# maturk/dn-splatter

Measured on NVIDIA H100. Metric: rendered Mpix/s (fwd+bwd, RGB+depth+normal), higher is better.
Workload: dtype f32

## Files before the change

dn_splatter_b200/csrc/adam.cu:

```cuda
#include "common.cuh"

namespace {

struct AdamSegDev {
  float* p; const float* g; float* m; float* v;
  int64_t n;
  float step_size, bc2_sqrt, eps;
};

struct AdamLaunch {
  AdamSegDev seg[DNR_ADAM_MAX_SEGS];
  float beta2, w1, w2;
};

__device__ __forceinline__ void adam_one(float& p, float g, float& m, float& v, float w1, float b2, float w2, float step_size,
                                         float bc2_sqrt, float eps) {
  m = m + w1 * (g - m);
  v = b2 * v + w2 * g * g;
  const float denom = sqrtf(v) / bc2_sqrt + eps;
  p = p - step_size * (m / denom);
}

__global__ void __launch_bounds__(256) adam_kernel(const AdamLaunch L) {
  const AdamSegDev& s = L.seg[blockIdx.y];
  const float w1 = L.w1, b2 = L.beta2, w2 = L.w2;
  const float step_size = s.step_size, bc2_sqrt = s.bc2_sqrt, eps = s.eps;
  const int64_t n = s.n;
  const int64_t tid = (int64_t)blockIdx.x * blockDim.x + threadIdx.x, stride = (int64_t)gridDim.x * blockDim.x;
  const bool vec = ((((uintptr_t)s.p | (uintptr_t)s.g | (uintptr_t)s.m | (uintptr_t)s.v) & 15) == 0);
  const int64_t n4 = vec ? (n >> 2) : 0;
  float4* p4 = reinterpret_cast<float4*>(s.p);
  const float4* g4 = reinterpret_cast<const float4*>(s.g);
  float4* m4 = reinterpret_cast<float4*>(s.m);
  float4* v4 = reinterpret_cast<float4*>(s.v);
  for (int64_t i = tid; i < n4; i += stride) {
    float4 p = p4[i], m = m4[i], v = v4[i];
    const float4 g = g4[i];
    adam_one(p.x, g.x, m.x, v.x, w1, b2, w2, step_size, bc2_sqrt, eps);
    adam_one(p.y, g.y, m.y, v.y, w1, b2, w2, step_size, bc2_sqrt, eps);
    adam_one(p.z, g.z, m.z, v.z, w1, b2, w2, step_size, bc2_sqrt, eps);
    adam_one(p.w, g.w, m.w, v.w, w1, b2, w2, step_size, bc2_sqrt, eps);
    p4[i] = p; m4[i] = m; v4[i] = v;
  }
  for (int64_t i = (n4 << 2) + tid; i < n; i += stride) {
    float p = s.p[i], m = s.m[i], v = s.v[i];
    adam_one(p, s.g[i], m, v, w1, b2, w2, step_size, bc2_sqrt, eps);
    s.p[i] = p; s.m[i] = m; s.v[i] = v;
  }
}

struct PeerDev {
  const float* flat[DNR_PEER_MAX];
  const uint8_t* touched[DNR_PEER_MAX];
  int world;
};

__global__ void __launch_bounds__(256) peer_mask_kernel(const PeerDev P, int n, uint8_t* __restrict__ mask) {
  const int i = (blockIdx.x * blockDim.x + threadIdx.x) * 16;
  if (i >= n) return;
  if (i + 16 <= n) {
    uint32_t m[4] = {0u, 0u, 0u, 0u};
    for (int k = 0; k < P.world; ++k) {
      const uint4 t = *reinterpret_cast<const uint4*>(P.touched[k] + i);
      const uint32_t w[4] = {t.x, t.y, t.z, t.w};
#pragma unroll
      for (int j = 0; j < 4; ++j) {
        const uint32_t nz = ((w[j] | ((w[j] & 0x7f7f7f7fu) + 0x7f7f7f7fu)) >> 7) & 0x01010101u;
        m[j] |= nz << k;
      }
    }
    *reinterpret_cast<uint4*>(mask + i) = make_uint4(m[0], m[1], m[2], m[3]);
  } else {
    for (int j = i; j < n; ++j) {
      uint32_t m = 0;
      for (int k = 0; k < P.world; ++k) m |= (P.touched[k][j] ? 1u : 0u) << k;
      mask[j] = (uint8_t)m;
    }
  }
}

struct AdamReduceLaunch {
  AdamLaunch adam;
  int dense[DNR_ADAM_MAX_SEGS];
  int64_t off[DNR_ADAM_MAX_SEGS];
  int32_t width[DNR_ADAM_MAX_SEGS];
};

template <int WORLD>
__global__ void __launch_bounds__(256, WORLD > 4 ? 3 : (WORLD > 1 ? 4 : 5)) adam_reduce_kernel(const AdamReduceLaunch L, const PeerDev P, const uint8_t* __restrict__ mask) {
  const AdamSegDev& s = L.adam.seg[blockIdx.y];
  const float w1 = L.adam.w1, b2 = L.adam.beta2, w2 = L.adam.w2;
  const float step_size = s.step_size, bc2_sqrt = s.bc2_sqrt, eps = s.eps;
  const int64_t n = s.n, off = L.off[blockIdx.y];
  const uint32_t width = (uint32_t)L.width[blockIdx.y];
  const uint32_t all_ranks = L.dense[blockIdx.y] ? ((1u << P.world) - 1u) : 0u;
  const int64_t tid = (int64_t)blockIdx.x * blockDim.x + threadIdx.x, stride = (int64_t)gridDim.x * blockDim.x;
  const int64_t n4 = n >> 2;
  float4* p4 = reinterpret_cast<float4*>(s.p);
  float4* m4 = reinterpret_cast<float4*>(s.m);
  float4* v4 = reinterpret_cast<float4*>(s.v);
  for (int64_t i = tid; i < n4; i += stride) {
    const uint32_t e = (uint32_t)(i << 2);
    uint32_t mk = all_ranks | (uint32_t)mask[e / width] | (uint32_t)mask[(e + 1u) / width] |
                  (uint32_t)mask[(e + 2u) / width] | (uint32_t)mask[(e + 3u) / width];
    if (WORLD == 1) mk = mk != 0u;
    float4 p = p4[i], m = m4[i], v = v4[i];
    float4 t[WORLD];
#pragma unroll
    for (int k = 0; k < WORLD; ++k) {
      t[k] = make_float4(0.f, 0.f, 0.f, 0.f);
      if ((mk >> k) & 1u) t[k] = reinterpret_cast<const float4*>(P.flat[k] + off)[i];
    }
    float4 g = t[0];
#pragma unroll
    for (int k = 1; k < WORLD; ++k) {
      g.x += t[k].x; g.y += t[k].y; g.z += t[k].z; g.w += t[k].w;
    }
    adam_one(p.x, g.x, m.x, v.x, w1, b2, w2, step_size, bc2_sqrt, eps);
    adam_one(p.y, g.y, m.y, v.y, w1, b2, w2, step_size, bc2_sqrt, eps);
    adam_one(p.z, g.z, m.z, v.z, w1, b2, w2, step_size, bc2_sqrt, eps);
    adam_one(p.w, g.w, m.w, v.w, w1, b2, w2, step_size, bc2_sqrt, eps);
    p4[i] = p; m4[i] = m; v4[i] = v;
  }
  for (int64_t i = (n4 << 2) + tid; i < n; i += stride) {
    uint32_t mk = all_ranks | (uint32_t)mask[(uint32_t)i / width];
    if (WORLD == 1) mk = mk != 0u;
    float g = 0.f;
    for (int k = 0; k < P.world; ++k)
      if ((mk >> k) & 1u) g += P.flat[k][off + i];
    float p = s.p[i], m = s.m[i], v = s.v[i];
    adam_one(p, g, m, v, w1, b2, w2, step_size, bc2_sqrt, eps);
    s.p[i] = p; s.m[i] = m; s.v[i] = v;
  }
}

struct GradZeroLaunch {
  float* g[DNR_ADAM_MAX_SEGS];
  int32_t width[DNR_ADAM_MAX_SEGS];
  int32_t dense[DNR_ADAM_MAX_SEGS];
  int n_segs;
};

constexpr int GZ_CHUNK = 256;

__global__ void __launch_bounds__(GZ_CHUNK) grad_zero_kernel(const GradZeroLaunch L, uint8_t* __restrict__ touched, int n) {
  __shared__ uint8_t s_f[GZ_CHUNK];
  const int tid = threadIdx.x;
  const int g0 = blockIdx.x * GZ_CHUNK;
  const int ng = min(GZ_CHUNK, n - g0);
  const uint8_t f = tid < ng ? touched[g0 + tid] : 0;
  s_f[tid] = f;
  const bool any = __syncthreads_or(f != 0);
  const float4 z = make_float4(0.f, 0.f, 0.f, 0.f);
  for (int s = 0; s < L.n_segs; ++s) {
    const bool dense = L.dense[s] != 0;
    if (!dense && !any) continue;
    const uint32_t w = (uint32_t)L.width[s];
    float4* out = reinterpret_cast<float4*>(L.g[s] + (size_t)g0 * w);
    const uint32_t n4 = ((uint32_t)ng * w + 3u) >> 2;
    for (uint32_t i = tid; i < n4; i += GZ_CHUNK) {
      bool hit = dense;
      if (!dense) {
        const uint32_t last = min((4u * i + 3u) / w, (uint32_t)ng - 1u);
        for (uint32_t j = (4u * i) / w; j <= last; ++j) hit |= s_f[j] != 0;
      }
      if (hit) out[i] = z;
    }
  }
  if (f) touched[g0 + tid] = 0;
}

}

static int fill_adam_launch(const DnrAdamSeg* segs, int32_t n_segs, double beta1, double beta2, AdamLaunch& L, int64_t& longest) {
  longest = 0;
  for (int i = 0; i < n_segs; ++i) {
    const DnrAdamSeg& s = segs[i];
    if (!s.p || !s.g || !s.m || !s.v) return DNR_E_NULL;
    if (s.n <= 0 || !(s.bc1 > 0.0) || !(s.bc2_sqrt > 0.0)) return DNR_E_SIZE;
    L.seg[i] = AdamSegDev{s.p, s.g, s.m, s.v, s.n, (float)(s.lr / s.bc1), (float)s.bc2_sqrt, (float)s.eps};
    longest = s.n > longest ? s.n : longest;
  }
  L.beta2 = (float)beta2;
  L.w1 = (float)(1.0 - beta1);
  L.w2 = (float)(1.0 - beta2);
  return 0;
}

extern "C" int dnr_adam_step_reduce(const DnrAdamSeg* segs, const int32_t* widths, int32_t n_segs, double beta1, double beta2,
                                    const DnrPeerReduce* peers, void* stream) {
  if (!segs || !widths || !peers) return DNR_E_NULL;
  if (n_segs <= 0 || n_segs > DNR_ADAM_MAX_SEGS) return DNR_E_SIZE;
  if (peers->world < 1 || peers->world > DNR_PEER_MAX || peers->rank < 0 || peers->rank >= peers->world || peers->n_gauss <= 0)
    return DNR_E_SIZE;
  if (!peers->mask && peers->world > 1) return DNR_E_NULL;
  AdamReduceLaunch L;
  int64_t longest = 0;
  if (const int rc = fill_adam_launch(segs, n_segs, beta1, beta2, L.adam, longest)) return rc;
  PeerDev P;
  P.world = peers->world;
  for (int k = 0; k < peers->world; ++k) {
    if (!peers->peer_flat[k] || !peers->peer_touched[k]) return DNR_E_NULL;
    P.flat[k] = peers->peer_flat[k];
    P.touched[k] = peers->peer_touched[k];
  }
  const float* mine = peers->peer_flat[peers->rank];
  for (int i = 0; i < n_segs; ++i) {
    if (widths[i] <= 0 || segs[i].n % widths[i] != 0 || segs[i].n / widths[i] != peers->n_gauss) return DNR_E_SIZE;
    if (segs[i].n >= ((int64_t)1 << 32)) return DNR_E_SIZE;
    L.off[i] = segs[i].g - mine;
    if (L.off[i] < 0 || (L.off[i] & 3) != 0) return DNR_E_SIZE;
    if (((uintptr_t)segs[i].p | (uintptr_t)segs[i].m | (uintptr_t)segs[i].v) & 15) return DNR_E_SIZE;
    L.width[i] = widths[i];
    L.dense[i] = segs[i].dense != 0;
  }
  cudaStream_t s = (cudaStream_t)stream;
  const int n = peers->n_gauss;
  if (peers->world > 1) {
    peer_mask_kernel<<<(n / 16 + 256) / 256, 256, 0, s>>>(P, n, peers->mask);
    DNR_CHECK_LAUNCH();
  }
  int64_t blocks = (longest / 4 + 255) / 256;
  if (blocks > DNR_NUM_SMS * 8) blocks = DNR_NUM_SMS * 8;
  if (blocks < 1) blocks = 1;
  const dim3 grid((unsigned)blocks, (unsigned)n_segs);
  if (peers->world == 1) adam_reduce_kernel<1><<<grid, 256, 0, s>>>(L, P, P.touched[0]);
  else if (peers->world <= 2) adam_reduce_kernel<2><<<grid, 256, 0, s>>>(L, P, peers->mask);
  else if (peers->world <= 4) adam_reduce_kernel<4><<<grid, 256, 0, s>>>(L, P, peers->mask);
  else adam_reduce_kernel<8><<<grid, 256, 0, s>>>(L, P, peers->mask);
  DNR_CHECK_LAUNCH();
  return 0;
}

extern "C" int dnr_adam_step(const DnrAdamSeg* segs, int32_t n_segs, double beta1, double beta2, void* stream) {
  if (!segs) return DNR_E_NULL;
  if (n_segs <= 0 || n_segs > DNR_ADAM_MAX_SEGS) return DNR_E_SIZE;
  AdamLaunch L;
  int64_t longest = 0;
  if (const int rc = fill_adam_launch(segs, n_segs, beta1, beta2, L, longest)) return rc;
  int64_t blocks = (longest / 4 + 255) / 256;
  if (blocks > DNR_NUM_SMS * 8) blocks = DNR_NUM_SMS * 8;
  if (blocks < 1) blocks = 1;
  adam_kernel<<<dim3((unsigned)blocks, (unsigned)n_segs), 256, 0, (cudaStream_t)stream>>>(L);
  DNR_CHECK_LAUNCH();
  return 0;
}

extern "C" int dnr_grad_zero(const DnrGradSeg* segs, int32_t n_segs, uint8_t* touched, int32_t n_gauss, void* stream) {
  if (!segs || !touched) return DNR_E_NULL;
  if (n_segs <= 0 || n_segs > DNR_ADAM_MAX_SEGS || n_gauss <= 0) return DNR_E_SIZE;
  GradZeroLaunch L;
  L.n_segs = n_segs;
  for (int i = 0; i < n_segs; ++i) {
    if (!segs[i].g) return DNR_E_NULL;
    if (segs[i].width <= 0 || segs[i].width > 4096 || ((uintptr_t)segs[i].g & 15)) return DNR_E_SIZE;
    L.g[i] = segs[i].g;
    L.width[i] = segs[i].width;
    L.dense[i] = segs[i].dense;
  }
  grad_zero_kernel<<<(n_gauss + GZ_CHUNK - 1) / GZ_CHUNK, GZ_CHUNK, 0, (cudaStream_t)stream>>>(L, touched, n_gauss);
  DNR_CHECK_LAUNCH();
  return 0;
}
```

dn_splatter_b200/csrc/binning.cu:

```cuda
#include <cub/cub.cuh>
#include <thrust/iterator/transform_iterator.h>

#include "common.cuh"

namespace {

inline size_t align_up(size_t x, size_t a = 256) { return (x + a - 1) / a * a; }

struct ToI64 {
  __host__ __device__ __forceinline__ int64_t operator()(int32_t v) const { return (int64_t)v; }
};

__global__ void iota_kernel(int32_t* out, int32_t n) {
  const int i = blockIdx.x * blockDim.x + threadIdx.x;
  if (i < n) out[i] = i;
}

struct ScanWs {
  uint32_t* keys_sorted;
  int32_t* order;
  int32_t* iota;
  int32_t* counts;
  int64_t* isect_start;
  void* cub_temp;
  size_t cub_bytes;
  size_t total;
};

ScanWs carve_scan(void* base, int32_t n) {
  ScanWs w;
  size_t off = 0;
  char* p = (char*)base;
  w.keys_sorted = (uint32_t*)(p + off); off += align_up((size_t)n * 4);
  w.order = (int32_t*)(p + off); off += align_up((size_t)n * 4);
  w.iota = (int32_t*)(p + off); off += align_up((size_t)n * 4);
  w.counts = (int32_t*)(p + off); off += align_up((size_t)(n + 1) * 4);
  w.isect_start = (int64_t*)(p + off); off += align_up((size_t)(n + 1) * 8);
  size_t sort_bytes = 0, scan_bytes = 0;
  cub::DeviceRadixSort::SortPairs(nullptr, sort_bytes, (const uint32_t*)nullptr, (uint32_t*)nullptr, (const int32_t*)nullptr,
                                  (int32_t*)nullptr, n, 0, 32);
  auto it = thrust::make_transform_iterator((const int32_t*)nullptr, ToI64());
  cub::DeviceScan::ExclusiveSum(nullptr, scan_bytes, it, (int64_t*)nullptr, n + 1);
  w.cub_bytes = sort_bytes > scan_bytes ? sort_bytes : scan_bytes;
  w.cub_temp = (void*)(p + off); off += align_up(w.cub_bytes);
  w.total = off;
  return w;
}

template <typename KeyT>
inline int sort_end_bit(int tile_bits) {
  const int full = (int)(8 * sizeof(KeyT));
  return tile_bits < full ? tile_bits : full;
}

template <typename KeyT>
struct SortWs {
  KeyT* keys_in;
  KeyT* keys_out;
  int32_t* gids_in;
  void* cub_temp;
  size_t cub_bytes;
  size_t total;
};

template <typename KeyT>
SortWs<KeyT> carve_sort(void* base, int64_t n_isects, int tile_bits) {
  SortWs<KeyT> w;
  size_t off = 0;
  char* p = (char*)base;
  const size_t n = (size_t)(n_isects > 0 ? n_isects : 1);
  w.keys_in = (KeyT*)(p + off); off += align_up(n * sizeof(KeyT));
  w.keys_out = (KeyT*)(p + off); off += align_up(n * sizeof(KeyT));
  w.gids_in = (int32_t*)(p + off); off += align_up(n * 4);
  size_t sort_bytes = 0;
  cub::DeviceRadixSort::SortPairs(nullptr, sort_bytes, (const KeyT*)nullptr, (KeyT*)nullptr, (const int32_t*)nullptr,
                                  (int32_t*)nullptr, (int64_t)n, 0, sort_end_bit<KeyT>(tile_bits));
  w.cub_bytes = sort_bytes;
  w.cub_temp = (void*)(p + off); off += align_up(sort_bytes);
  w.total = off;
  return w;
}

inline int tile_bits_for(int n_tiles) {
  int b = 1;
  while ((1 << b) <= n_tiles) ++b;
  return b;
}

struct HitGauss {
  int g, radius, x0, y0, nx, ny;
  float mx, my, A, B, invA, bac, twoAL, ex_max, ey_max, ey_star;
};

__device__ __forceinline__ void list_box(float mx, float my, int radius, int ts, int tiles_x, int tiles_y, int& x0, int& y0,
                                         int& x1, int& y1) {
  if (ts == DNR_TILE) { dnr_tile_box(mx, my, radius, tiles_x, tiles_y, x0, y0, x1, y1); return; }
  const float inv = 1.0f / (float)ts;
  const float r = (float)radius * inv, tcx = mx * inv, tcy = my * inv;
  x0 = min(max((int)floorf(tcx - r), 0), tiles_x);
  y0 = min(max((int)floorf(tcy - r), 0), tiles_y);
  x1 = min(max((int)ceilf(tcx + r), 0), tiles_x);
  y1 = min(max((int)ceilf(tcy + r), 0), tiles_y);
}

__device__ __forceinline__ HitGauss load_hit_gauss(const DnrArgs& a, const int32_t* __restrict__ order, int i, int tiles_x,
                                                   int tiles_y) {
  HitGauss h;
  h.g = 0; h.radius = 0; h.x0 = h.y0 = h.nx = h.ny = 0;
  h.mx = h.my = h.A = h.B = h.invA = h.bac = h.twoAL = h.ex_max = h.ey_max = h.ey_star = 0.f;
  if (i < a.n_gauss) {
    h.g = order[i];
    h.radius = a.radii[h.g];
    if (h.radius > 0) {
      h.mx = a.means2d[h.g * 2 + 0]; h.my = a.means2d[h.g * 2 + 1];
      int x1, y1;
      list_box(h.mx, h.my, h.radius, DNR_TILE << a.list_shift, tiles_x, tiles_y, h.x0, h.y0, x1, y1);
      h.nx = x1 - h.x0;
      h.ny = y1 - h.y0;
      if (!(a.flags & DNR_FLAG_EXACT_LISTS)) {
        const float A = a.conics[h.g * 3 + 0], B = a.conics[h.g * 3 + 1], C = a.conics[h.g * 3 + 2];
        const float L = a.cull_lim[h.g];
        const float det = A * C - B * B;
        if (!(L > 0.f) || !(det > 0.f)) {
          h.ny = 0;
        } else {
          h.A = A; h.B = B; h.invA = 1.0f / A; h.bac = -det; h.twoAL = 2.0f * A * L;
          h.ex_max = sqrtf(2.0f * L * C / det) * 1.0001f + 0.01f;
          h.ey_max = sqrtf(2.0f * L * A / det) * 1.0001f + 0.01f;
          h.ey_star = -B * h.ex_max / C;
        }
      }
    }
  }
  return h;
}

__device__ __forceinline__ void row_span(const HitGauss& h, int ty, bool exact, int ts, int& lo, int& hi) {
  lo = h.x0; hi = h.x0 + h.nx;
  if (exact) return;
  float e0 = ((float)(ty * ts) + 0.5f) - h.my - 0.01f;
  float e1 = ((float)(ty * ts + ts - 1) + 0.5f) - h.my + 0.01f;
  if (e0 > h.ey_max || e1 < -h.ey_max) { hi = lo; return; }
  e0 = fmaxf(e0, -h.ey_max); e1 = fminf(e1, h.ey_max);
  const float s0 = sqrtf(fmaxf(fmaf(h.bac, e0 * e0, h.twoAL), 0.f)), s1 = sqrtf(fmaxf(fmaf(h.bac, e1 * e1, h.twoAL), 0.f));
  float xmax = fmaxf((-h.B * e0 + s0) * h.invA, (-h.B * e1 + s1) * h.invA);
  float xmin = fminf((-h.B * e0 - s0) * h.invA, (-h.B * e1 - s1) * h.invA);
  if (h.ey_star >= e0 && h.ey_star <= e1) xmax = h.ex_max;
  if (-h.ey_star >= e0 && -h.ey_star <= e1) xmin = -h.ex_max;
  xmax = xmax + 0.01f + 1e-5f * fabsf(xmax);
  xmin = xmin - 0.01f - 1e-5f * fabsf(xmin);
  const float inv = 1.0f / (float)ts;
  const int t_lo = (int)ceilf((h.mx + xmin - ((float)ts - 0.5f)) * inv);
  const int t_hi = (int)floorf((h.mx + xmax - 0.5f) * inv) + 1;
  lo = max(lo, t_lo); hi = min(hi, t_hi);
}

__global__ void __launch_bounds__(256) count_kernel(const DnrArgs a, const int32_t* __restrict__ order,
                                                   int32_t* __restrict__ counts, int tiles_x, int tiles_y) {
  const int i = blockIdx.x * blockDim.x + threadIdx.x;
  if (i > a.n_gauss) return;
  const HitGauss h = load_hit_gauss(a, order, i, tiles_x, tiles_y);
  const bool exact = (a.flags & DNR_FLAG_EXACT_LISTS) != 0;
  const int ts = DNR_TILE << a.list_shift;
  int cnt = 0;
  for (int r = 0; r < h.ny; ++r) {
    int lo, hi;
    row_span(h, h.y0 + r, exact, ts, lo, hi);
    cnt += max(hi - lo, 0);
  }
  counts[i] = (i < a.n_gauss) ? cnt : 0;
}

template <typename KeyT>
__global__ void __launch_bounds__(256) emit_kernel(const DnrArgs a, const int32_t* __restrict__ order,
                                                  const int64_t* __restrict__ isect_start, KeyT* __restrict__ keys,
                                                  int32_t* __restrict__ gids, int tiles_x, int tiles_y) {
  const int i = blockIdx.x * blockDim.x + threadIdx.x;
  if (i >= a.n_gauss) return;
  int64_t dst = isect_start[i];
  const int64_t dst_end = isect_start[i + 1];
  if (dst_end <= dst) return;
  const HitGauss h = load_hit_gauss(a, order, i, tiles_x, tiles_y);
  const int64_t cap = a.n_isects;
  const bool exact = (a.flags & DNR_FLAG_EXACT_LISTS) != 0;
  const int ts = DNR_TILE << a.list_shift;
  for (int r = 0; r < h.ny; ++r) {
    int lo, hi;
    row_span(h, h.y0 + r, exact, ts, lo, hi);
    const int row_key = (h.y0 + r) * tiles_x;
    for (int x = lo; x < hi; ++x, ++dst) {
      if (dst < cap) {
        keys[dst] = (KeyT)(row_key + x);
        gids[dst] = h.g;
      }
    }
  }
}

template <typename KeyT>
__global__ void __launch_bounds__(256) pad_kernel(KeyT* __restrict__ keys, int32_t* __restrict__ gids,
                                                 const int64_t* __restrict__ n_isects_dev, int64_t cap, KeyT pad_key) {
  for (int64_t i = *n_isects_dev + (int64_t)blockIdx.x * blockDim.x + threadIdx.x; i < cap; i += (int64_t)gridDim.x * blockDim.x) {
    keys[i] = pad_key;
    gids[i] = 0;
  }
}

template <typename KeyT>
__global__ void __launch_bounds__(256) offsets_kernel(const KeyT* __restrict__ keys, const int64_t* __restrict__ n_isects_dev,
                                                     int64_t cap, int n_tiles, int32_t* __restrict__ offsets) {
  const int64_t i = (int64_t)blockIdx.x * blockDim.x + threadIdx.x;
  const int64_t n_isects = min(*n_isects_dev, cap);
  if (n_isects == 0) {
    if (i <= n_tiles) offsets[i] = 0;
    return;
  }
  if (i >= n_isects) return;
  const int cur = (int)keys[i];
  if (i == 0) {
    for (int t = 0; t <= cur; ++t) offsets[t] = 0;
  } else {
    const int prev = (int)keys[i - 1];
    for (int t = prev + 1; t <= cur; ++t) offsets[t] = (int32_t)i;
  }
  if (i == n_isects - 1) {
    for (int t = cur + 1; t <= n_tiles; ++t) offsets[t] = (int32_t)n_isects;
  }
}

template <typename KeyT>
int bin_sort_impl(const DnrArgs* a, cudaStream_t s, int n_tiles, int tile_bits) {
  const int tiles_x = dnr_stiles_x(a), tiles_y = dnr_stiles_y(a);
  ScanWs sw = carve_scan(a->ws_scan, a->n_gauss);
  const int64_t cap = a->n_isects;
  SortWs<KeyT> w = carve_sort<KeyT>(a->ws_sort, cap, tile_bits);
  if (cap > 0) {
    emit_kernel<KeyT><<<(unsigned)((a->n_gauss + 255) / 256), 256, 0, s>>>(*a, sw.order, sw.isect_start, w.keys_in, w.gids_in,
                                                                          tiles_x, tiles_y);
    DNR_CHECK_LAUNCH();
    pad_kernel<KeyT><<<DNR_NUM_SMS * 2, 256, 0, s>>>(w.keys_in, w.gids_in, a->n_isects_dev, cap, (KeyT)n_tiles);
    DNR_CHECK_LAUNCH();
    size_t bytes = w.cub_bytes;
    const int end_bit = sort_end_bit<KeyT>(tile_bits);
    DNR_CUDA(cub::DeviceRadixSort::SortPairs(w.cub_temp, bytes, (const KeyT*)w.keys_in, w.keys_out,
                                             (const int32_t*)w.gids_in, a->flatten_ids, cap, 0, end_bit, s));
  }
  const int64_t n = cap > (int64_t)n_tiles + 1 ? cap : (int64_t)n_tiles + 1;
  offsets_kernel<KeyT><<<(unsigned)((n + 255) / 256), 256, 0, s>>>(w.keys_out, a->n_isects_dev, cap, n_tiles, a->tile_offsets);
  DNR_CHECK_LAUNCH();
  return 0;
}

}

extern "C" size_t dnr_bin_scan_workspace_bytes(int32_t n_gauss) {
  if (n_gauss <= 0) return 0;
  return carve_scan(nullptr, n_gauss).total;
}

extern "C" int dnr_bin_scan(const DnrArgs* a, void* stream, int64_t* n_isects_host) {
  if (!a) return DNR_E_NULL;
  if (a->n_gauss <= 0 || a->width <= 0 || a->height <= 0) return DNR_E_SIZE;
  if (a->list_shift < 0 || a->list_shift > 3) return DNR_E_OPTION;
  if ((a->flags & DNR_FLAG_EXACT_LISTS) && a->list_shift != 0) return DNR_E_OPTION;
  if (!a->ws_scan || !a->depth_keys || !a->tiles_per_gauss || !a->n_isects_dev || !a->radii || !a->means2d) return DNR_E_NULL;
  if (!(a->flags & DNR_FLAG_EXACT_LISTS) && (!a->conics || !a->cull_lim)) return DNR_E_NULL;
  cudaStream_t s = (cudaStream_t)stream;
  const int32_t n = a->n_gauss;
  ScanWs w = carve_scan(a->ws_scan, n);
  iota_kernel<<<(n + 255) / 256, 256, 0, s>>>(w.iota, n);
  DNR_CHECK_LAUNCH();
  size_t bytes = w.cub_bytes;
  DNR_CUDA(cub::DeviceRadixSort::SortPairs(w.cub_temp, bytes, (const uint32_t*)a->depth_keys, w.keys_sorted,
                                           (const int32_t*)w.iota, w.order, n, 0, 32, s));
  {
    const int64_t threads = (int64_t)n + 1;
    count_kernel<<<(unsigned)((threads + 255) / 256), 256, 0, s>>>(*a, w.order, w.counts, dnr_stiles_x(a), dnr_stiles_y(a));
    DNR_CHECK_LAUNCH();
  }
  auto it = thrust::make_transform_iterator((const int32_t*)w.counts, ToI64());
  bytes = w.cub_bytes;
  DNR_CUDA(cub::DeviceScan::ExclusiveSum(w.cub_temp, bytes, it, w.isect_start, n + 1, s));
  DNR_CUDA(cudaMemcpyAsync(a->n_isects_dev, w.isect_start + n, sizeof(int64_t), cudaMemcpyDeviceToDevice, s));
  if (n_isects_host) {
    int64_t total = 0;
    DNR_CUDA(cudaMemcpyAsync(&total, w.isect_start + n, sizeof(int64_t), cudaMemcpyDeviceToHost, s));
    DNR_CUDA(cudaStreamSynchronize(s));
    *n_isects_host = total;
    if (total > 0x7FFFFFFFLL) return DNR_E_OVERFLOW;
  }
  return 0;
}

extern "C" size_t dnr_bin_sort_workspace_bytes(int32_t n_gauss, int64_t n_isects, int32_t n_tiles) {
  (void)n_gauss;
  if (n_isects < 0 || n_tiles <= 0) return 0;
  const int bits = tile_bits_for(n_tiles);
  if (n_tiles < 65536) return carve_sort<uint16_t>(nullptr, n_isects, bits).total;
  return carve_sort<uint32_t>(nullptr, n_isects, bits).total;
}

extern "C" int dnr_bin_sort(const DnrArgs* a, void* stream) {
  if (!a) return DNR_E_NULL;
  if (a->n_gauss <= 0 || a->n_isects < 0 || a->width <= 0 || a->height <= 0) return DNR_E_SIZE;
  if (a->n_isects > 0x7FFFFFFFLL) return DNR_E_OVERFLOW;
  if (!a->ws_scan || !a->ws_sort || !a->tile_offsets || !a->means2d || !a->radii || !a->n_isects_dev) return DNR_E_NULL;
  if (!(a->flags & DNR_FLAG_EXACT_LISTS) && (!a->conics || !a->cull_lim)) return DNR_E_NULL;
  if (a->n_isects > 0 && !a->flatten_ids) return DNR_E_NULL;
  if (a->list_shift < 0 || a->list_shift > 3) return DNR_E_OPTION;
  if ((a->flags & DNR_FLAG_EXACT_LISTS) && a->list_shift != 0) return DNR_E_OPTION;
  const int n_tiles = dnr_stiles_x(a) * dnr_stiles_y(a);
  const int bits = tile_bits_for(n_tiles);
  cudaStream_t s = (cudaStream_t)stream;
  if (n_tiles < 65536) return bin_sort_impl<uint16_t>(a, s, n_tiles, bits);
  return bin_sort_impl<uint32_t>(a, s, n_tiles, bits);
}
```

Measured before the change: 774.9.

## Flatten Adam segments into one 1-D grid, use magic division, compact grad-zero

After: 784.7 (median of 6 runs). +1.3%, better.

```diff
diff --git a/dn_splatter_b200/csrc/adam.cu b/dn_splatter_b200/csrc/adam.cu
--- a/dn_splatter_b200/csrc/adam.cu
+++ b/dn_splatter_b200/csrc/adam.cu
@@ -1,4 +1,8 @@
 #include "common.cuh"
+
+#define DNR_DIV_MAX_W 4096
+static inline uint64_t dnr_div_magic(uint32_t w) { return ((uint64_t(1) << 44) + w - 1u) / w; }
+__device__ __forceinline__ uint32_t dnr_div(uint32_t e, uint64_t m) { return (uint32_t)__umul64hi((uint64_t)e << 20, m); }
 
 namespace {
 
@@ -83,91 +87,158 @@
   AdamLaunch adam;
   int dense[DNR_ADAM_MAX_SEGS];
   int64_t off[DNR_ADAM_MAX_SEGS];
-  int32_t width[DNR_ADAM_MAX_SEGS];
-};
+  uint64_t wdiv[DNR_ADAM_MAX_SEGS];
+  int64_t start4[DNR_ADAM_MAX_SEGS + 1];
+  int n_segs;
+};
+
+template <int WORLD> struct AdamReduceShape {
+  static constexpr int batch = WORLD == 1 ? 3 : (WORLD <= 4 ? 2 : 1);
+  static constexpr int ctas_per_sm = 3;
+};
+constexpr int ADAM_THREADS = 256;
 
 template <int WORLD>
-__global__ void __launch_bounds__(256, WORLD > 4 ? 3 : (WORLD > 1 ? 4 : 5)) adam_reduce_kernel(const AdamReduceLaunch L, const PeerDev P, const uint8_t* __restrict__ mask) {
-  const AdamSegDev& s = L.adam.seg[blockIdx.y];
+__global__ void __launch_bounds__(ADAM_THREADS, AdamReduceShape<WORLD>::ctas_per_sm)
+    adam_reduce_kernel(const AdamReduceLaunch L, const PeerDev P, const uint8_t* __restrict__ mask) {
+  constexpr int U = AdamReduceShape<WORLD>::batch;
   const float w1 = L.adam.w1, b2 = L.adam.beta2, w2 = L.adam.w2;
-  const float step_size = s.step_size, bc2_sqrt = s.bc2_sqrt, eps = s.eps;
-  const int64_t n = s.n, off = L.off[blockIdx.y];
-  const uint32_t width = (uint32_t)L.width[blockIdx.y];
-  const uint32_t all_ranks = L.dense[blockIdx.y] ? ((1u << P.world) - 1u) : 0u;
-  const int64_t tid = (int64_t)blockIdx.x * blockDim.x + threadIdx.x, stride = (int64_t)gridDim.x * blockDim.x;
-  const int64_t n4 = n >> 2;
-  float4* p4 = reinterpret_cast<float4*>(s.p);
-  float4* m4 = reinterpret_cast<float4*>(s.m);
-  float4* v4 = reinterpret_cast<float4*>(s.v);
-  for (int64_t i = tid; i < n4; i += stride) {
-    const uint32_t e = (uint32_t)(i << 2);
-    uint32_t mk = all_ranks | (uint32_t)mask[e / width] | (uint32_t)mask[(e + 1u) / width] |
-                  (uint32_t)mask[(e + 2u) / width] | (uint32_t)mask[(e + 3u) / width];
-    if (WORLD == 1) mk = mk != 0u;
-    float4 p = p4[i], m = m4[i], v = v4[i];
-    float4 t[WORLD];
-#pragma unroll
-    for (int k = 0; k < WORLD; ++k) {
-      t[k] = make_float4(0.f, 0.f, 0.f, 0.f);
-      if ((mk >> k) & 1u) t[k] = reinterpret_cast<const float4*>(P.flat[k] + off)[i];
-    }
-    float4 g = t[0];
-#pragma unroll
-    for (int k = 1; k < WORLD; ++k) {
-      g.x += t[k].x; g.y += t[k].y; g.z += t[k].z; g.w += t[k].w;
-    }
-    adam_one(p.x, g.x, m.x, v.x, w1, b2, w2, step_size, bc2_sqrt, eps);
-    adam_one(p.y, g.y, m.y, v.y, w1, b2, w2, step_size, bc2_sqrt, eps);
-    adam_one(p.z, g.z, m.z, v.z, w1, b2, w2, step_size, bc2_sqrt, eps);
-    adam_one(p.w, g.w, m.w, v.w, w1, b2, w2, step_size, bc2_sqrt, eps);
-    p4[i] = p; m4[i] = m; v4[i] = v;
-  }
-  for (int64_t i = (n4 << 2) + tid; i < n; i += stride) {
-    uint32_t mk = all_ranks | (uint32_t)mask[(uint32_t)i / width];
-    if (WORLD == 1) mk = mk != 0u;
-    float g = 0.f;
-    for (int k = 0; k < P.world; ++k)
-      if ((mk >> k) & 1u) g += P.flat[k][off + i];
-    float p = s.p[i], m = s.m[i], v = s.v[i];
-    adam_one(p, g, m, v, w1, b2, w2, step_size, bc2_sqrt, eps);
-    s.p[i] = p; s.m[i] = m; s.v[i] = v;
-  }
+  const uint32_t all_ranks = (1u << P.world) - 1u;
+  const int64_t hi = L.start4[L.n_segs];
+  int s = 0;
+  for (int64_t base = (int64_t)blockIdx.x * ADAM_THREADS * U + threadIdx.x; base < hi;
+       base += (int64_t)gridDim.x * ADAM_THREADS * U) {
+    int seg[U];
+    uint32_t f[U], mk[U];
+#pragma unroll
+    for (int k = 0; k < U; ++k) {
+      const int64_t F = base + k * ADAM_THREADS;
+      mk[k] = 0u;
+      f[k] = 0u;
+      seg[k] = s;
+      if (F >= hi) continue;
+      while (F >= L.start4[s + 1]) ++s;
+      seg[k] = s;
+      f[k] = (uint32_t)(F - L.start4[s]);
+      if (L.dense[s]) {
+        mk[k] = all_ranks;
+      } else {
+        const uint64_t wd = L.wdiv[s];
+        const uint32_t a = dnr_div(f[k] << 2, wd), b = dnr_div((f[k] << 2) + 3u, wd);
+        mk[k] = (uint32_t)mask[a] | (uint32_t)mask[min(a + 1u, b)] | (uint32_t)mask[min(a + 2u, b)] | (uint32_t)mask[b];
+        if (WORLD == 1) mk[k] = mk[k] != 0u;
+      }
+    }
+    float4 p[U], m[U], v[U], g[U];
+#pragma unroll
+    for (int k = 0; k < U; ++k) {
+      const bool live = base + k * ADAM_THREADS < hi;
+      const AdamSegDev& sd = L.adam.seg[seg[k]];
+      if (live) {
+        p[k] = reinterpret_cast<const float4*>(sd.p)[f[k]];
+        m[k] = reinterpret_cast<const float4*>(sd.m)[f[k]];
+        v[k] = reinterpret_cast<const float4*>(sd.v)[f[k]];
+      }
+    }
+#pragma unroll
+    for (int k = 0; k < U; ++k) {
+      const int64_t off = L.off[seg[k]];
+      float4 t[WORLD];
+#pragma unroll
+      for (int r = 0; r < WORLD; ++r) {
+        t[r] = make_float4(0.f, 0.f, 0.f, 0.f);
+        if ((mk[k] >> r) & 1u) t[r] = reinterpret_cast<const float4*>(P.flat[r] + off)[f[k]];
+      }
+      g[k] = t[0];
+#pragma unroll
+      for (int r = 1; r < WORLD; ++r) {
+        g[k].x += t[r].x; g[k].y += t[r].y; g[k].z += t[r].z; g[k].w += t[r].w;
+      }
+    }
+#pragma unroll
+    for (int k = 0; k < U; ++k) {
+      if (base + k * ADAM_THREADS >= hi) continue;
+      const AdamSegDev& sd = L.adam.seg[seg[k]];
+      const float step_size = sd.step_size, bc2_sqrt = sd.bc2_sqrt, eps = sd.eps;
+      adam_one(p[k].x, g[k].x, m[k].x, v[k].x, w1, b2, w2, step_size, bc2_sqrt, eps);
+      adam_one(p[k].y, g[k].y, m[k].y, v[k].y, w1, b2, w2, step_size, bc2_sqrt, eps);
+      adam_one(p[k].z, g[k].z, m[k].z, v[k].z, w1, b2, w2, step_size, bc2_sqrt, eps);
+      adam_one(p[k].w, g[k].w, m[k].w, v[k].w, w1, b2, w2, step_size, bc2_sqrt, eps);
+      reinterpret_cast<float4*>(sd.p)[f[k]] = p[k];
+      reinterpret_cast<float4*>(sd.m)[f[k]] = m[k];
+      reinterpret_cast<float4*>(sd.v)[f[k]] = v[k];
+    }
+  }
+  const int t = blockIdx.x * ADAM_THREADS + threadIdx.x;
+  if (t >= 4 * L.n_segs) return;
+  s = t >> 2;
+  const AdamSegDev& sd = L.adam.seg[s];
+  const int64_t i = ((sd.n >> 2) << 2) + (t & 3);
+  if (i >= sd.n) return;
+  uint32_t mk = L.dense[s] ? all_ranks : (uint32_t)mask[dnr_div((uint32_t)i, L.wdiv[s])];
+  if (WORLD == 1) mk = mk != 0u;
+  float g = 0.f;
+  for (int k = 0; k < P.world; ++k)
+    if ((mk >> k) & 1u) g += P.flat[k][L.off[s] + i];
+  float p = sd.p[i], m = sd.m[i], v = sd.v[i];
+  adam_one(p, g, m, v, w1, b2, w2, sd.step_size, sd.bc2_sqrt, sd.eps);
+  sd.p[i] = p; sd.m[i] = m; sd.v[i] = v;
 }
 
 struct GradZeroLaunch {
   float* g[DNR_ADAM_MAX_SEGS];
-  int32_t width[DNR_ADAM_MAX_SEGS];
+  uint32_t width[DNR_ADAM_MAX_SEGS];
   int32_t dense[DNR_ADAM_MAX_SEGS];
   int n_segs;
 };
 
-constexpr int GZ_CHUNK = 256;
-
-__global__ void __launch_bounds__(GZ_CHUNK) grad_zero_kernel(const GradZeroLaunch L, uint8_t* __restrict__ touched, int n) {
-  __shared__ uint8_t s_f[GZ_CHUNK];
-  const int tid = threadIdx.x;
+constexpr int GZ_THREADS = 256, GZ_CHUNK = 1024;
+
+__global__ void __launch_bounds__(GZ_THREADS) grad_zero_kernel(const GradZeroLaunch L, uint8_t* __restrict__ touched, int n) {
+  __shared__ uint16_t s_list[GZ_CHUNK];
+  __shared__ int s_count;
+  const int tid = threadIdx.x, lane = tid & 31, warp = tid >> 5;
   const int g0 = blockIdx.x * GZ_CHUNK;
   const int ng = min(GZ_CHUNK, n - g0);
-  const uint8_t f = tid < ng ? touched[g0 + tid] : 0;
-  s_f[tid] = f;
-  const bool any = __syncthreads_or(f != 0);
+  if (tid == 0) s_count = 0;
+  __syncthreads();
+  if (tid < GZ_CHUNK / 16) {
+    const int j = 16 * tid;
+    uint8_t* src = touched + g0 + j;
+    if (j + 16 <= ng && ((uintptr_t)src & 15) == 0) {
+      const uint4 f = *reinterpret_cast<const uint4*>(src);
+      if (f.x | f.y | f.z | f.w) {
+        *reinterpret_cast<uint4*>(src) = make_uint4(0u, 0u, 0u, 0u);
+        const uint32_t w[4] = {f.x, f.y, f.z, f.w};
+#pragma unroll
+        for (int b = 0; b < 16; ++b)
+          if ((w[b >> 2] >> (8 * (b & 3))) & 0xffu) s_list[atomicAdd(&s_count, 1)] = (uint16_t)(j + b);
+      }
+    } else {
+      for (int b = 0; b < 16 && j + b < ng; ++b) {
+        if (src[b]) {
+          src[b] = 0;
+          s_list[atomicAdd(&s_count, 1)] = (uint16_t)(j + b);
+        }
+      }
+    }
+  }
+  __syncthreads();
+  const int count = s_count;
   const float4 z = make_float4(0.f, 0.f, 0.f, 0.f);
   for (int s = 0; s < L.n_segs; ++s) {
-    const bool dense = L.dense[s] != 0;
-    if (!dense && !any) continue;
-    const uint32_t w = (uint32_t)L.width[s];
-    float4* out = reinterpret_cast<float4*>(L.g[s] + (size_t)g0 * w);
-    const uint32_t n4 = ((uint32_t)ng * w + 3u) >> 2;
-    for (uint32_t i = tid; i < n4; i += GZ_CHUNK) {
-      bool hit = dense;
-      if (!dense) {
-        const uint32_t last = min((4u * i + 3u) / w, (uint32_t)ng - 1u);
-        for (uint32_t j = (4u * i) / w; j <= last; ++j) hit |= s_f[j] != 0;
-      }
-      if (hit) out[i] = z;
-    }
-  }
-  if (f) touched[g0 + tid] = 0;
+    const int64_t w = L.width[s];
+    float4* out = reinterpret_cast<float4*>(L.g[s]);
+    if (L.dense[s]) {
+      const int64_t a = (g0 * w) >> 2, b = ((g0 + ng) * w + 3) >> 2;
+      for (int64_t q = a + tid; q < b; q += GZ_THREADS) out[q] = z;
+      continue;
+    }
+    for (int r = warp; r < count; r += GZ_THREADS / 32) {
+      const int64_t e = (g0 + s_list[r]) * w;
+      for (int64_t q = (e >> 2) + lane; q <= (e + w - 1) >> 2; q += 32) out[q] = z;
+    }
+  }
 }
 
 }
@@ -205,29 +276,40 @@
     P.touched[k] = peers->peer_touched[k];
   }
   const float* mine = peers->peer_flat[peers->rank];
+  int64_t total4 = 0;
   for (int i = 0; i < n_segs; ++i) {
-    if (widths[i] <= 0 || segs[i].n % widths[i] != 0 || segs[i].n / widths[i] != peers->n_gauss) return DNR_E_SIZE;
+    if (widths[i] <= 0 || widths[i] > DNR_DIV_MAX_W || segs[i].n % widths[i] != 0 || segs[i].n / widths[i] != peers->n_gauss)
+      return DNR_E_SIZE;
     if (segs[i].n >= ((int64_t)1 << 32)) return DNR_E_SIZE;
     L.off[i] = segs[i].g - mine;
     if (L.off[i] < 0 || (L.off[i] & 3) != 0) return DNR_E_SIZE;
     if (((uintptr_t)segs[i].p | (uintptr_t)segs[i].m | (uintptr_t)segs[i].v) & 15) return DNR_E_SIZE;
-    L.width[i] = widths[i];
+    L.wdiv[i] = dnr_div_magic((uint32_t)widths[i]);
     L.dense[i] = segs[i].dense != 0;
-  }
+    L.start4[i] = total4;
+    total4 += segs[i].n >> 2;
+  }
+  L.start4[n_segs] = total4;
+  L.n_segs = n_segs;
   cudaStream_t s = (cudaStream_t)stream;
   const int n = peers->n_gauss;
   if (peers->world > 1) {
     peer_mask_kernel<<<(n / 16 + 256) / 256, 256, 0, s>>>(P, n, peers->mask);
     DNR_CHECK_LAUNCH();
   }
-  int64_t blocks = (longest / 4 + 255) / 256;
-  if (blocks > DNR_NUM_SMS * 8) blocks = DNR_NUM_SMS * 8;
-  if (blocks < 1) blocks = 1;
-  const dim3 grid((unsigned)blocks, (unsigned)n_segs);
-  if (peers->world == 1) adam_reduce_kernel<1><<<grid, 256, 0, s>>>(L, P, P.touched[0]);
-  else if (peers->world <= 2) adam_reduce_kernel<2><<<grid, 256, 0, s>>>(L, P, peers->mask);
-  else if (peers->world <= 4) adam_reduce_kernel<4><<<grid, 256, 0, s>>>(L, P, peers->mask);
-  else adam_reduce_kernel<8><<<grid, 256, 0, s>>>(L, P, peers->mask);
+  auto grid = [&](auto shape) {
+    const int64_t tile = ADAM_THREADS * decltype(shape)::batch, slots = DNR_NUM_SMS * decltype(shape)::ctas_per_sm;
+    const int64_t blocks = (total4 + tile - 1) / tile;
+    return (unsigned)(blocks < 1 ? 1 : (blocks > slots ? slots : blocks));
+  };
+  if (peers->world == 1)
+    adam_reduce_kernel<1><<<grid(AdamReduceShape<1>{}), ADAM_THREADS, 0, s>>>(L, P, P.touched[0]);
+  else if (peers->world <= 2)
+    adam_reduce_kernel<2><<<grid(AdamReduceShape<2>{}), ADAM_THREADS, 0, s>>>(L, P, peers->mask);
+  else if (peers->world <= 4)
+    adam_reduce_kernel<4><<<grid(AdamReduceShape<4>{}), ADAM_THREADS, 0, s>>>(L, P, peers->mask);
+  else
+    adam_reduce_kernel<8><<<grid(AdamReduceShape<8>{}), ADAM_THREADS, 0, s>>>(L, P, peers->mask);
   DNR_CHECK_LAUNCH();
   return 0;
 }
@@ -253,12 +335,12 @@
   L.n_segs = n_segs;
   for (int i = 0; i < n_segs; ++i) {
     if (!segs[i].g) return DNR_E_NULL;
-    if (segs[i].width <= 0 || segs[i].width > 4096 || ((uintptr_t)segs[i].g & 15)) return DNR_E_SIZE;
+    if (segs[i].width <= 0 || segs[i].width > DNR_DIV_MAX_W || ((uintptr_t)segs[i].g & 15)) return DNR_E_SIZE;
     L.g[i] = segs[i].g;
-    L.width[i] = segs[i].width;
+    L.width[i] = (uint32_t)segs[i].width;
     L.dense[i] = segs[i].dense;
   }
-  grad_zero_kernel<<<(n_gauss + GZ_CHUNK - 1) / GZ_CHUNK, GZ_CHUNK, 0, (cudaStream_t)stream>>>(L, touched, n_gauss);
+  grad_zero_kernel<<<(n_gauss + GZ_CHUNK - 1) / GZ_CHUNK, GZ_THREADS, 0, (cudaStream_t)stream>>>(L, touched, n_gauss);
   DNR_CHECK_LAUNCH();
   return 0;
 }
```

## Count tiles in gaussian order and cache packed gaussian inputs for emit

Applied to the files above, without the earlier changes.

Result: no change. 774.5 before, 778.6 after (median of 6 runs) (+0.5%).

```diff
diff --git a/dn_splatter_b200/csrc/binning.cu b/dn_splatter_b200/csrc/binning.cu
--- a/dn_splatter_b200/csrc/binning.cu
+++ b/dn_splatter_b200/csrc/binning.cu
@@ -1,4 +1,5 @@
 #include <cub/cub.cuh>
+#include <thrust/iterator/counting_iterator.h>
 #include <thrust/iterator/transform_iterator.h>
 
 #include "common.cuh"
@@ -7,9 +8,20 @@
 
 inline size_t align_up(size_t x, size_t a = 256) { return (x + a - 1) / a * a; }
 
-struct ToI64 {
-  __host__ __device__ __forceinline__ int64_t operator()(int32_t v) const { return (int64_t)v; }
-};
+struct __align__(16) GaussIn {
+  int32_t radius;
+  float mx, my, A, B, C, L, pad;
+};
+
+struct DepthOrderCount {
+  const int32_t* counts;
+  const int32_t* order;
+  int32_t n;
+  __host__ __device__ __forceinline__ int64_t operator()(int32_t i) const {
+    return i < n ? (int64_t)counts[order[i]] : 0;
+  }
+};
+using DepthOrderCounts = thrust::transform_iterator<DepthOrderCount, thrust::counting_iterator<int32_t>, int64_t>;
 
 __global__ void iota_kernel(int32_t* out, int32_t n) {
   const int i = blockIdx.x * blockDim.x + threadIdx.x;
@@ -21,6 +33,7 @@
   int32_t* order;
   int32_t* iota;
   int32_t* counts;
+  GaussIn* gauss;
   int64_t* isect_start;
   void* cub_temp;
   size_t cub_bytes;
@@ -34,12 +47,13 @@
   w.keys_sorted = (uint32_t*)(p + off); off += align_up((size_t)n * 4);
   w.order = (int32_t*)(p + off); off += align_up((size_t)n * 4);
   w.iota = (int32_t*)(p + off); off += align_up((size_t)n * 4);
-  w.counts = (int32_t*)(p + off); off += align_up((size_t)(n + 1) * 4);
+  w.counts = (int32_t*)(p + off); off += align_up((size_t)n * 4);
+  w.gauss = (GaussIn*)(p + off); off += align_up((size_t)n * sizeof(GaussIn));
   w.isect_start = (int64_t*)(p + off); off += align_up((size_t)(n + 1) * 8);
   size_t sort_bytes = 0, scan_bytes = 0;
   cub::DeviceRadixSort::SortPairs(nullptr, sort_bytes, (const uint32_t*)nullptr, (uint32_t*)nullptr, (const int32_t*)nullptr,
                                   (int32_t*)nullptr, n, 0, 32);
-  auto it = thrust::make_transform_iterator((const int32_t*)nullptr, ToI64());
+  DepthOrderCounts it(thrust::counting_iterator<int32_t>(0), DepthOrderCount{nullptr, nullptr, n});
   cub::DeviceScan::ExclusiveSum(nullptr, scan_bytes, it, (int64_t*)nullptr, n + 1);
   w.cub_bytes = sort_bytes > scan_bytes ? sort_bytes : scan_bytes;
   w.cub_temp = (void*)(p + off); off += align_up(w.cub_bytes);
@@ -103,32 +117,41 @@
   y1 = min(max((int)ceilf(tcy + r), 0), tiles_y);
 }
 
-__device__ __forceinline__ HitGauss load_hit_gauss(const DnrArgs& a, const int32_t* __restrict__ order, int i, int tiles_x,
-                                                   int tiles_y) {
+__device__ __forceinline__ GaussIn load_gauss(const DnrArgs& a, int g) {
+  GaussIn in;
+  in.radius = a.radii[g];
+  in.mx = in.my = in.A = in.B = in.C = in.L = in.pad = 0.f;
+  if (in.radius > 0) {
+    in.mx = a.means2d[g * 2 + 0]; in.my = a.means2d[g * 2 + 1];
+    if (!(a.flags & DNR_FLAG_EXACT_LISTS)) {
+      in.A = a.conics[g * 3 + 0]; in.B = a.conics[g * 3 + 1]; in.C = a.conics[g * 3 + 2];
+      in.L = a.cull_lim[g];
+    }
+  }
+  return in;
+}
+
+__device__ __forceinline__ HitGauss hit_gauss(const DnrArgs& a, int g, const GaussIn& in, int tiles_x, int tiles_y) {
   HitGauss h;
-  h.g = 0; h.radius = 0; h.x0 = h.y0 = h.nx = h.ny = 0;
+  h.g = g; h.radius = in.radius; h.x0 = h.y0 = h.nx = h.ny = 0;
   h.mx = h.my = h.A = h.B = h.invA = h.bac = h.twoAL = h.ex_max = h.ey_max = h.ey_star = 0.f;
-  if (i < a.n_gauss) {
-    h.g = order[i];
-    h.radius = a.radii[h.g];
-    if (h.radius > 0) {
-      h.mx = a.means2d[h.g * 2 + 0]; h.my = a.means2d[h.g * 2 + 1];
-      int x1, y1;
-      list_box(h.mx, h.my, h.radius, DNR_TILE << a.list_shift, tiles_x, tiles_y, h.x0, h.y0, x1, y1);
-      h.nx = x1 - h.x0;
-      h.ny = y1 - h.y0;
-      if (!(a.flags & DNR_FLAG_EXACT_LISTS)) {
-        const float A = a.conics[h.g * 3 + 0], B = a.conics[h.g * 3 + 1], C = a.conics[h.g * 3 + 2];
-        const float L = a.cull_lim[h.g];
-        const float det = A * C - B * B;
-        if (!(L > 0.f) || !(det > 0.f)) {
-          h.ny = 0;
-        } else {
-          h.A = A; h.B = B; h.invA = 1.0f / A; h.bac = -det; h.twoAL = 2.0f * A * L;
-          h.ex_max = sqrtf(2.0f * L * C / det) * 1.0001f + 0.01f;
-          h.ey_max = sqrtf(2.0f * L * A / det) * 1.0001f + 0.01f;
-          h.ey_star = -B * h.ex_max / C;
-        }
+  if (h.radius > 0) {
+    h.mx = in.mx; h.my = in.my;
+    int x1, y1;
+    list_box(h.mx, h.my, h.radius, DNR_TILE << a.list_shift, tiles_x, tiles_y, h.x0, h.y0, x1, y1);
+    h.nx = x1 - h.x0;
+    h.ny = y1 - h.y0;
+    if (!(a.flags & DNR_FLAG_EXACT_LISTS)) {
+      const float A = in.A, B = in.B, C = in.C;
+      const float L = in.L;
+      const float det = A * C - B * B;
+      if (!(L > 0.f) || !(det > 0.f)) {
+        h.ny = 0;
+      } else {
+        h.A = A; h.B = B; h.invA = 1.0f / A; h.bac = -det; h.twoAL = 2.0f * A * L;
+        h.ex_max = sqrtf(2.0f * L * C / det) * 1.0001f + 0.01f;
+        h.ey_max = sqrtf(2.0f * L * A / det) * 1.0001f + 0.01f;
+        h.ey_star = -B * h.ex_max / C;
       }
     }
   }
@@ -155,11 +178,12 @@
   lo = max(lo, t_lo); hi = min(hi, t_hi);
 }
 
-__global__ void __launch_bounds__(256) count_kernel(const DnrArgs a, const int32_t* __restrict__ order,
-                                                   int32_t* __restrict__ counts, int tiles_x, int tiles_y) {
-  const int i = blockIdx.x * blockDim.x + threadIdx.x;
-  if (i > a.n_gauss) return;
-  const HitGauss h = load_hit_gauss(a, order, i, tiles_x, tiles_y);
+__global__ void __launch_bounds__(256) count_kernel(const DnrArgs a, int32_t* __restrict__ counts,
+                                                   GaussIn* __restrict__ gauss, int tiles_x, int tiles_y) {
+  const int g = blockIdx.x * blockDim.x + threadIdx.x;
+  if (g >= a.n_gauss) return;
+  const GaussIn in = load_gauss(a, g);
+  const HitGauss h = hit_gauss(a, g, in, tiles_x, tiles_y);
   const bool exact = (a.flags & DNR_FLAG_EXACT_LISTS) != 0;
   const int ts = DNR_TILE << a.list_shift;
   int cnt = 0;
@@ -168,11 +192,13 @@
     row_span(h, h.y0 + r, exact, ts, lo, hi);
     cnt += max(hi - lo, 0);
   }
-  counts[i] = (i < a.n_gauss) ? cnt : 0;
+  counts[g] = cnt;
+  if (cnt > 0) gauss[g] = in;
 }
 
 template <typename KeyT>
 __global__ void __launch_bounds__(256) emit_kernel(const DnrArgs a, const int32_t* __restrict__ order,
+                                                  const GaussIn* __restrict__ gauss,
                                                   const int64_t* __restrict__ isect_start, KeyT* __restrict__ keys,
                                                   int32_t* __restrict__ gids, int tiles_x, int tiles_y) {
   const int i = blockIdx.x * blockDim.x + threadIdx.x;
@@ -180,7 +206,8 @@
   int64_t dst = isect_start[i];
   const int64_t dst_end = isect_start[i + 1];
   if (dst_end <= dst) return;
-  const HitGauss h = load_hit_gauss(a, order, i, tiles_x, tiles_y);
+  const int g = order[i];
+  const HitGauss h = hit_gauss(a, g, gauss[g], tiles_x, tiles_y);
   const int64_t cap = a.n_isects;
   const bool exact = (a.flags & DNR_FLAG_EXACT_LISTS) != 0;
   const int ts = DNR_TILE << a.list_shift;
@@ -235,7 +262,7 @@
   const int64_t cap = a->n_isects;
   SortWs<KeyT> w = carve_sort<KeyT>(a->ws_sort, cap, tile_bits);
   if (cap > 0) {
-    emit_kernel<KeyT><<<(unsigned)((a->n_gauss + 255) / 256), 256, 0, s>>>(*a, sw.order, sw.isect_start, w.keys_in, w.gids_in,
+    emit_kernel<KeyT><<<(unsigned)((a->n_gauss + 255) / 256), 256, 0, s>>>(*a, sw.order, sw.gauss, sw.isect_start, w.keys_in, w.gids_in,
                                                                           tiles_x, tiles_y);
     DNR_CHECK_LAUNCH();
     pad_kernel<KeyT><<<DNR_NUM_SMS * 2, 256, 0, s>>>(w.keys_in, w.gids_in, a->n_isects_dev, cap, (KeyT)n_tiles);
@@ -273,12 +300,9 @@
   size_t bytes = w.cub_bytes;
   DNR_CUDA(cub::DeviceRadixSort::SortPairs(w.cub_temp, bytes, (const uint32_t*)a->depth_keys, w.keys_sorted,
                                            (const int32_t*)w.iota, w.order, n, 0, 32, s));
-  {
-    const int64_t threads = (int64_t)n + 1;
-    count_kernel<<<(unsigned)((threads + 255) / 256), 256, 0, s>>>(*a, w.order, w.counts, dnr_stiles_x(a), dnr_stiles_y(a));
-    DNR_CHECK_LAUNCH();
-  }
-  auto it = thrust::make_transform_iterator((const int32_t*)w.counts, ToI64());
+  count_kernel<<<(unsigned)((n + 255) / 256), 256, 0, s>>>(*a, w.counts, w.gauss, dnr_stiles_x(a), dnr_stiles_y(a));
+  DNR_CHECK_LAUNCH();
+  DepthOrderCounts it(thrust::counting_iterator<int32_t>(0), DepthOrderCount{w.counts, w.order, n});
   bytes = w.cub_bytes;
   DNR_CUDA(cub::DeviceScan::ExclusiveSum(w.cub_temp, bytes, it, w.isect_start, n + 1, s));
   DNR_CUDA(cudaMemcpyAsync(a->n_isects_dev, w.isect_start + n, sizeof(int64_t), cudaMemcpyDeviceToDevice, s));
```
